# AtomGradient/swift-qwen3-tts

Measured on AMD Instinct MI355X. Metric: codec_tokens_per_s, higher is better.
Workload: dtype bf16

## Files before the change

swift-qwen3-tts_amd/csrc/debug_env.cc:

```cpp
#include <atomic>
#include <cstdlib>
#include <mutex>

#include "kernels.h"

namespace q3 {

namespace {
std::mutex g_mu;
std::atomic<const DebugEnv*> g_env{nullptr};

bool flag(const char* name) { return std::getenv(name) != nullptr; }
int number(const char* name, int dflt) {
    const char* e = std::getenv(name);
    return e && *e ? std::atoi(e) : dflt;
}

const DebugEnv* read_env() {
    DebugEnv* d = new DebugEnv{};
    d->gemm_no_row_split = flag("Q3TTS_GEMM_NO_ROW_SPLIT");
    d->gemm_one_pair = flag("Q3TTS_GEMM_ONE_PAIR");
    d->gemm_parent_forms = number("Q3TTS_GEMM_PARENT_FORMS", 0) != 0;
    d->no_tall_gemm = flag("Q3TTS_NO_TALL_GEMM");
    d->tall_shape = number("Q3TTS_TALL_SHAPE", 0);
    d->chunk_qsplit = number("Q3TTS_CHUNK_QSPLIT", 0);
    d->conv_no_pw = flag("Q3TTS_CONV_NO_PW");
    d->nt_off = std::getenv("Q3TTS_NT") && number("Q3TTS_NT", 1) == 0;
    d->serial_jobs = number("Q3TTS_SERIAL_JOBS", 0) != 0;
    d->fail_back_half = number("Q3TTS_TEST_FAIL_BACK_HALF", 0) != 0;
    d->no_prefix_cache = number("Q3TTS_NO_PREFIX_CACHE", 0) != 0;
    return d;
}
}

const DebugEnv& debug_env() {
    const DebugEnv* e = g_env.load(std::memory_order_acquire);
    if (!e) {
        std::lock_guard<std::mutex> lk(g_mu);
        e = g_env.load(std::memory_order_acquire);
        if (!e) {
            e = read_env();
            g_env.store(e, std::memory_order_release);
        }
    }
    return *e;
}

void debug_env_reload() {
    std::lock_guard<std::mutex> lk(g_mu);
    g_env.store(read_env(), std::memory_order_release);
}

}
```

swift-qwen3-tts_amd/csrc/kernels.h:

```cpp
#pragma once
#include <hip/hip_runtime.h>

#include <cstdint>

namespace q3 {

struct DebugEnv {
    bool gemm_no_row_split;
    bool gemm_one_pair;
    bool gemm_parent_forms;
    bool no_tall_gemm;
    int tall_shape;
    int chunk_qsplit;
    bool conv_no_pw;
    bool nt_off;
    bool serial_jobs;
    bool fail_back_half;
    bool no_prefix_cache;
};
const DebugEnv& debug_env();
void debug_env_reload();

constexpr int kPageTokens = 64;
constexpr int kHeadDim = 128;

struct NormRowsArgs {
    const uint16_t* h;
    int hMB;
    const uint16_t* w;
    float eps;
    uint16_t* out;
    int outMB;
    float* ss_out;
    int M, H;
    const float* ss_in;
    int ss_count, ss_ld;
};
void launch_norm_rows(const NormRowsArgs& a, hipStream_t st);

struct GemmArgs {
    const uint16_t* W;
    const uint32_t* Wsb;
    const uint16_t* x;
    int xMB;
    int M, Mpad, N, K;
    int epi;
    uint16_t* y;
    int ldy;
    int y_tiled, yMB;
    const uint16_t* bias;
    int act_silu;
    const uint16_t* norm_w;
    const float* ss_in;
    int ss_count, ss_ld, norm_dim;
    float norm_eps;
    int nt_weights;
    int resid;
    float* ss_out;
};
void launch_gemm_skinny(const GemmArgs& a, hipStream_t st);
struct SkinnyGeom {
    bool tall;
    int split, mbw;
    int nw, ch, np;
    int gx;
    bool ntw;
    bool tm;
// ... 189 lines not shown
```

swift-qwen3-tts_amd/csrc/kernels/codec_conv.hip:

```cpp
#include <cstdlib>
#include <mutex>

#include "../common.h"
#include "../codec_kernels.h"
#include "../kernels.h"
#include "snake.h"

namespace q3 {
namespace {

constexpr int BM = 128;
constexpr int KC = 32;
constexpr int LDS_LD = 40;
constexpr int MAX_HALO = 56;

__device__ __forceinline__ void st16(float* p, const float4& v) { *reinterpret_cast<float4*>(p) = v; }
__device__ __forceinline__ float4 ld16f(const float* p) { return *reinterpret_cast<const float4*>(p); }

__device__ __forceinline__ float gelu_erf(float v) { return 0.5f * v * (1.0f + erff(v * 0.70710678118654752440f)); }

__device__ __forceinline__ float act_other(float v, int act) {
    switch (act) {
        case 2: return v * 0.5f * (1.0f + tanhf(0.7978845608f * (v + 0.044715f * (v * v * v))));
        case 3: return fmaxf(v, 0.f);
// ... 231 lines not shown
                    for (int c = 0; c < CT; ++c) acc[p][c] = __builtin_amdgcn_mfma_f32_16x16x4f32(wa[g][c].x, xa[g][p].x, acc[p][c], 0, 0, 0);
#pragma unroll
                for (int p = 0; p < 4; ++p)
#pragma unroll
                    for (int c = 0; c < CT; ++c) acc[p][c] = __builtin_amdgcn_mfma_f32_16x16x4f32(wa[g][c].y, xa[g][p].y, acc[p][c], 0, 0, 0);
#pragma unroll
                for (int p = 0; p < 4; ++p)
#pragma unroll
                    for (int c = 0; c < CT; ++c) acc[p][c] = __builtin_amdgcn_mfma_f32_16x16x4f32(wa[g][c].z, xa[g][p].z, acc[p][c], 0, 0, 0);
#pragma unroll
                for (int p = 0; p < 4; ++p)
#pragma unroll
                    for (int c = 0; c < CT; ++c) acc[p][c] = __builtin_amdgcn_mfma_f32_16x16x4f32(wa[g][c].w, xa[g][p].w, acc[p][c], 0, 0, 0);
            }
            buf ^= 1;
        }
    }

    epilogue_tile<CT, true>(a, b, t0 + wm * 64, n0 + wn * (BN / 2), T, lane, acc);
    if (a.out2) snake_pass<CT>(a, smem, b, t0, n0, wn, T, wave, lane, acc, wm);
}

constexpr int ROWH = 40;

typedef _Float16 f16x8 __attribute__((ext_vector_type(8)));
typedef _Float16 f16x4 __attribute__((ext_vector_type(4)));
typedef float f32x4v __attribute__((ext_vector_type(4)));

__device__ __forceinline__ void split_h2(const float4& v, uint2& hi, uint2& lo) {
    const f32x4v x = {v.x, v.y, v.z, v.w};
    const f16x4 h = __builtin_convertvector(x, f16x4);
    const f32x4v r = (x - __builtin_convertvector(h, f32x4v)) * 2048.0f;
    const f16x4 l = __builtin_convertvector(r, f16x4);
    __builtin_memcpy(&hi, &h, 8);
    __builtin_memcpy(&lo, &l, 8);
}

__device__ __forceinline__ f32x4 mfma_f16(const uint4& a, const uint4& b, f32x4 c) {
    f16x8 av, bv;
    __builtin_memcpy(&av, &a, 16);
    __builtin_memcpy(&bv, &b, 16);
    return __builtin_amdgcn_mfma_f32_16x16x32_f16(av, bv, c, 0, 0, 0);
}

__device__ __forceinline__ uint4 f16x8_scale_m11(const uint4& a) {
    f16x8 v;
    __builtin_memcpy(&v, &a, 16);
    v = v * static_cast<_Float16>(0.00048828125f);
    uint4 r;
    __builtin_memcpy(&r, &v, 16);
    return r;
}

template <int CT>
__device__ __forceinline__ void scale_acc(const float* wsc, int N, int n_w, int lane, f32x4 (&acc)[4][CT]) {
    const int nq = n_w + 4 * (lane >> 4);
#pragma unroll
    for (int c = 0; c < CT; ++c) {
        const int n = nq + 16 * c;
        float4 s = make_float4(1.f, 1.f, 1.f, 1.f);
        if (n < N) s = *reinterpret_cast<const float4*>(wsc + n);
#pragma unroll
        for (int p = 0; p < 4; ++p) {
            acc[p][c][0] *= s.x; acc[p][c][1] *= s.y; acc[p][c][2] *= s.z; acc[p][c][3] *= s.w;
        }
    }
}

template <int BN, bool PRO>
__global__ __launch_bounds__(256, 2) void conv_gemm_h2_kernel(ConvGemmArgs a) {
    constexpr int CT = BN / 32;
    extern __shared__ __attribute__((aligned(16))) uint32_t smem3[];
    const int halo = (a.K - 1) * a.dil;
    uint32_t* As = smem3;
    uint32_t* Ws = smem3 + (BM + halo) * ROWH;

    const int tid = threadIdx.x, lane = tid & 63, wave = tid >> 6;
    const int wm = wave >> 1, wn = wave & 1;
    int b, n_tile, m_tile;
    {
        const uint32_t gx = gridDim.x, gy = gridDim.y, nwg = gx * gy * gridDim.z;
        const uint32_t bid = blockIdx.x + gx * (blockIdx.y + gy * blockIdx.z);
        const uint32_t q = nwg >> 3, r = nwg & 7u, xcd = bid & 7u;
        const uint32_t swz = (xcd < r ? xcd * (q + 1) : r * (q + 1) + (xcd - r) * q) + (bid >> 3);
        n_tile = int(swz % gx);
        const uint32_t rest = swz / gx;
        m_tile = int(rest % gy);
        b = int(rest / gy);
    }
    const int n0 = n_tile * BN;
    const int t0 = m_tile * BM;
    const int T = a.frames[b] * a.ppf;
    if (t0 >= T) return;
    const int rows = BM + halo;
    const float* xb = a.x + (size_t)b * a.x_bstride;
    const float* x2b = a.x2;
    const int nchunks = (a.Cin + KC - 1) / KC;
    const int steps = nchunks * a.K;

    f32x4 acc[4][CT];
#pragma unroll
    for (int p = 0; p < 4; ++p)
#pragma unroll
        for (int c = 0; c < CT; ++c) acc[p][c] = f32x4{0.f, 0.f, 0.f, 0.f};

    constexpr int WV = BN * 8 / 256;
    uint4 wreg[WV];
    auto load_w = [&](int step) {
        const int chunk = step / a.K, tap = step % a.K;
        const uint4* src = reinterpret_cast<const uint4*>(a.wh + ((size_t)(tap * nchunks + chunk) * a.N + n0) * 64);
#pragma unroll
        for (int i = 0; i < WV; ++i) {
            const int item = i * 256 + tid;
            uint4 v = make_uint4(0u, 0u, 0u, 0u);
            if (n0 + (item >> 3) < a.N) v = src[item];
            wreg[i] = v;
        }
    };
    auto store_w = [&](int buf) {
#pragma unroll
        for (int i = 0; i < WV; ++i) {
            const int item = i * 256 + tid;
// ... 6 lines not shown
    auto load_a = [&](int chunk) {
        const int c0 = chunk * KC;
#pragma unroll
        for (int i = 0; i < AV; ++i) {
            const int item = i * 256 + tid;
            const int r = item >> 3, c4 = (item & 7) * 4;
            int t = t0 - halo + r;
            if constexpr (PRO) {
                t += a.shift;
                if (a.reflect) t = t < 0 ? -t : (t >= T ? 2 * (T - 1) - t : t);
            }
            float4 v = make_float4(0.f, 0.f, 0.f, 0.f);
            if (r < rows && t >= -a.hist && t < T && c0 + c4 < a.Cin) {
                v = ld16f(xb + (int64_t)t * a.ldx + c0 + c4);
                if constexpr (PRO) {
                    if (x2b) {
                        const float4 u = *reinterpret_cast<const float4*>(x2b + (int64_t)t * a.ldx2 + c0 + c4);
                        v.x += u.x; v.y += u.y; v.z += u.z; v.w += u.w;
                    }
                    if (a.pre_act == 1) {
                        v.x = v.x > 0.f ? v.x : expf(v.x) - 1.0f;
                        v.y = v.y > 0.f ? v.y : expf(v.y) - 1.0f;
                        v.z = v.z > 0.f ? v.z : expf(v.z) - 1.0f;
                        v.w = v.w > 0.f ? v.w : expf(v.w) - 1.0f;
                    }
                    if (a.snake_ea) {
                        const float4 ea = *reinterpret_cast<const float4*>(a.snake_ea + c0 + c4);
                        const float4 ib = *reinterpret_cast<const float4*>(a.snake_ib + c0 + c4);
                        float s;
                        s = sinf(v.x * ea.x); v.x = v.x + ib.x * (s * s);
                        s = sinf(v.y * ea.y); v.y = v.y + ib.y * (s * s);
                        s = sinf(v.z * ea.z); v.z = v.z + ib.z * (s * s);
                        s = sinf(v.w * ea.w); v.w = v.w + ib.w * (s * s);
                    }
                }
            }
            areg[i] = v;
        }
    };
    auto store_a = [&]() {
#pragma unroll
        for (int i = 0; i < AV; ++i) {
            const int item = i * 256 + tid;
            const int r = item >> 3, c4 = (item & 7) * 4;
            if (r >= rows) continue;
            uint2 hi, lo;
            split_h2(areg[i], hi, lo);
            uint32_t* dst = &As[r * ROWH + (c4 >> 1)];
            *reinterpret_cast<uint2*>(dst) = hi;
            *reinterpret_cast<uint2*>(dst + 16) = lo;
        }
    };

    load_w(0);
    load_a(0);
    int buf = 0;
    for (int chunk = 0; chunk < nchunks; ++chunk) {
        __syncthreads();
        store_a();
        if (chunk + 1 < nchunks) load_a(chunk + 1);
        for (int tap = 0; tap < a.K; ++tap) {
            const int step = chunk * a.K + tap;
            store_w(buf);
            __syncthreads();
            if (step + 1 < steps) load_w(step + 1);
            const uint32_t* arow = &As[(wm * 64 + tap * a.dil + (lane & 15)) * ROWH + 4 * (lane >> 4)];
            const uint32_t* wrow = &Ws[(buf * BN + wn * (BN / 2) + (lane & 15)) * ROWH + 4 * (lane >> 4)];
            uint4 xa[2][4], wa[2][CT], wb[CT];
#pragma unroll
            for (int pl = 0; pl < 2; ++pl) {
#pragma unroll
                for (int p = 0; p < 4; ++p) xa[pl][p] = *reinterpret_cast<const uint4*>(arow + p * 16 * ROWH + pl * 16);
#pragma unroll
                for (int c = 0; c < CT; ++c) wa[pl][c] = *reinterpret_cast<const uint4*>(wrow + c * 16 * ROWH + pl * 16);
            }
#pragma unroll
            for (int c = 0; c < CT; ++c) wb[c] = f16x8_scale_m11(wa[0][c]);
#pragma unroll
            for (int p = 0; p < 4; ++p)
#pragma unroll
                for (int c = 0; c < CT; ++c) acc[p][c] = mfma_f16(wb[c], xa[1][p], acc[p][c]);
#pragma unroll
            for (int p = 0; p < 4; ++p)
#pragma unroll
                for (int c = 0; c < CT; ++c) acc[p][c] = mfma_f16(wa[1][c], xa[0][p], acc[p][c]);
#pragma unroll
            for (int p = 0; p < 4; ++p)
#pragma unroll
                for (int c = 0; c < CT; ++c) acc[p][c] = mfma_f16(wa[0][c], xa[0][p], acc[p][c]);
            buf ^= 1;
        }
    }

    scale_acc<CT>(a.wsc, a.N, n0 + wn * (BN / 2), lane, acc);
    if (a.act != 0) epilogue_tile<CT, true>(a, b, t0 + wm * 64, n0 + wn * (BN / 2), T, lane, acc);
    else epilogue_tile<CT, false>(a, b, t0 + wm * 64, n0 + wn * (BN / 2), T, lane, acc);
    if (a.out2) snake_pass<CT>(a, reinterpret_cast<float*>(smem3), b, t0, n0, wn, T, wave, lane, acc, wm);
}

template <int BN, int D>
__global__ __launch_bounds__(256, 2) void conv_pw_h2_kernel(ConvGemmArgs a) {
    constexpr int CT = BN / 32;
    constexpr int WV = BN * 8 / 256, AV = BM * 8 / 256;
    using u32x4 = __attribute__((ext_vector_type(4))) uint32_t;
    using f32x4r = __attribute__((ext_vector_type(4))) float;
    extern __shared__ __attribute__((aligned(16))) uint32_t smem3[];
    uint32_t* As = smem3;
    uint32_t* Ws = smem3 + BM * ROWH;

    const int tid = threadIdx.x, lane = tid & 63, wave = tid >> 6;
    const int wm = wave >> 1, wn = wave & 1;
    int b, n_tile, m_tile;
    {
        const uint32_t gx = gridDim.x, gy = gridDim.y, nwg = gx * gy * gridDim.z;
        const uint32_t bid = blockIdx.x + gx * (blockIdx.y + gy * blockIdx.z);
        const uint32_t q = nwg >> 3, r = nwg & 7u, xcd = bid & 7u;
        const uint32_t swz = (xcd < r ? xcd * (q + 1) : r * (q + 1) + (xcd - r) * q) + (bid >> 3);
        n_tile = int(swz % gx);
        const uint32_t rest = swz / gx;
        m_tile = int(rest % gy);
        b = int(rest / gy);
    }
    const int n0 = n_tile * BN, t0 = m_tile * BM;
    const int T = a.frames[b] * a.ppf;
    if (t0 >= T) return;
    const float* xb = a.x + (size_t)b * a.x_bstride;
    const int steps = (a.Cin + KC - 1) / KC;

    f32x4 acc[4][CT];
#pragma unroll
    for (int p = 0; p < 4; ++p)
#pragma unroll
        for (int c = 0; c < CT; ++c) acc[p][c] = f32x4{0.f, 0.f, 0.f, 0.f};

    const float* asrc[AV];
    bool aok[AV];
#pragma unroll
    for (int i = 0; i < AV; ++i) {
        const int item = i * 256 + tid, r = item >> 3;
        const int t = t0 + r;
        aok[i] = t >= -a.hist && t < T;
        const int tc = t < T ? t : T - 1;
        asrc[i] = xb + (int64_t)tc * a.ldx + (item & 7) * 4;
    }
// ... 35 lines not shown
        _Pragma("unroll") for (int i = 0; i < WV; ++i) {                                          \
            const int item = i * 256 + tid;                                                       \
            *reinterpret_cast<u32x4*>(&Ws[(item >> 3) * ROWH + (item & 7) * 4]) = rw[J][i];       \
        }                                                                                         \
    }
#define Q3_PW_STEP(J, GUARD)                                                                      \
    if (!(GUARD) || s0 + (J) < steps) {                                                           \
        __syncthreads();                     \
        Q3_PW_STORE(J, s0 + (J))                                                                  \
        __builtin_amdgcn_sched_barrier(0);                                                        \
        { const int nx_ = s0 + (J) + D; Q3_PW_LOAD(J, nx_ < steps ? nx_ : steps - 1) }            \
        __builtin_amdgcn_sched_barrier(0);                                                        \
        __syncthreads();                                                                          \
        const uint32_t* arow = &As[(wm * 64 + (lane & 15)) * ROWH + 4 * (lane >> 4)];             \
        const uint32_t* wrow = &Ws[(wn * (BN / 2) + (lane & 15)) * ROWH + 4 * (lane >> 4)];       \
        uint4 xa[2][4], wa[2][CT], wb[CT];                                                        \
        _Pragma("unroll") for (int pl = 0; pl < 2; ++pl) {                                        \
            _Pragma("unroll") for (int p = 0; p < 4; ++p) xa[pl][p] = *reinterpret_cast<const uint4*>(arow + p * 16 * ROWH + pl * 16); \
            _Pragma("unroll") for (int c = 0; c < CT; ++c) wa[pl][c] = *reinterpret_cast<const uint4*>(wrow + c * 16 * ROWH + pl * 16); \
        }                                                                                         \
        _Pragma("unroll") for (int c = 0; c < CT; ++c) wb[c] = f16x8_scale_m11(wa[0][c]);         \
        _Pragma("unroll") for (int p = 0; p < 4; ++p)                                             \
            _Pragma("unroll") for (int c = 0; c < CT; ++c) acc[p][c] = mfma_f16(wb[c], xa[1][p], acc[p][c]);    \
        _Pragma("unroll") for (int p = 0; p < 4; ++p)                                             \
            _Pragma("unroll") for (int c = 0; c < CT; ++c) acc[p][c] = mfma_f16(wa[1][c], xa[0][p], acc[p][c]); \
        _Pragma("unroll") for (int p = 0; p < 4; ++p)                                             \
            _Pragma("unroll") for (int c = 0; c < CT; ++c) acc[p][c] = mfma_f16(wa[0][c], xa[0][p], acc[p][c]); \
    }
#define Q3_PW_GROUP(G)                                       \
    Q3_PW_STEP(0, G) Q3_PW_STEP(1, G)                        \
    if constexpr (D > 2) { Q3_PW_STEP(2, G) }                \
    if constexpr (D > 3) { Q3_PW_STEP(3, G) }

    Q3_PW_LOAD(0, 0)
    __builtin_amdgcn_sched_barrier(0);
    Q3_PW_LOAD(1, 1 < steps ? 1 : steps - 1)
    __builtin_amdgcn_sched_barrier(0);
    if constexpr (D > 2) { Q3_PW_LOAD(2, 2 < steps ? 2 : steps - 1) __builtin_amdgcn_sched_barrier(0); }
    if constexpr (D > 3) { Q3_PW_LOAD(3, 3 < steps ? 3 : steps - 1) __builtin_amdgcn_sched_barrier(0); }
    int s0 = 0;
    for (; s0 + D <= steps; s0 += D) { Q3_PW_GROUP(false) }
    if (s0 < steps) { Q3_PW_GROUP(true) }
#undef Q3_PW_GROUP
#undef Q3_PW_STEP
#undef Q3_PW_STORE
#undef Q3_PW_LOAD

    scale_acc<CT>(a.wsc, a.N, n0 + wn * (BN / 2), lane, acc);
    if (a.act != 0) epilogue_tile<CT, true>(a, b, t0 + wm * 64, n0 + wn * (BN / 2), T, lane, acc);
    else epilogue_tile<CT, false>(a, b, t0 + wm * 64, n0 + wn * (BN / 2), T, lane, acc);
    if (a.out2) snake_pass<CT>(a, reinterpret_cast<float*>(smem3), b, t0, n0, wn, T, wave, lane, acc, wm);
}

template <int CT2, int PT>
__global__ __launch_bounds__(256, 2) void resunit_h2_kernel(ResUnitArgs a) {
    constexpr int C = 16 * CT2, NCH = CT2 / 2, PW = 16 * PT, BMU = 4 * PW;
    constexpr int CG = CT2 >= 12 ? 4 : (CT2 == 6 ? 3 : CT2);
    constexpr int NG = CT2 / CG;
    static_assert(CT2 % CG == 0 && CT2 % 2 == 0, "channel tiles must split into groups and into 32-channel chunks");
    extern __shared__ __attribute__((aligned(16))) uint32_t smem3[];
    const int halo = (a.K - 1) * a.dil;
    uint32_t* As = smem3;
    uint32_t* Ws = smem3 + (BMU + halo) * ROWH;
    const bool wdb = a.wdb != 0;

    const int tid = threadIdx.x, lane = tid & 63, wave = tid >> 6;
    const int b = blockIdx.z;
    const int t0 = blockIdx.y * BMU;
    const int T = a.frames[b] * a.ppf;
    if (t0 >= T) return;
    const int rows = BMU + halo;
    const size_t boff = (size_t)b * a.Tmax * C;
    const float* yb = a.y + boff;
    const int S1 = NCH * a.K;

    f32x4 acc1[PT][CT2];
#pragma unroll
    for (int p = 0; p < PT; ++p)
#pragma unroll
        for (int c = 0; c < CT2; ++c) acc1[p][c] = f32x4{0.f, 0.f, 0.f, 0.f};

    constexpr int WV = (C * 8 + 255) / 256;
    uint4 wreg[WV];
    auto load_w = [&](int step) {
        const uint4* src;
        int items;
        if (step < S1) {
            const int chunk = step / a.K, tap = step % a.K;
            src = reinterpret_cast<const uint4*>(a.w1h + (size_t)(tap * NCH + chunk) * C * 64);
            items = C * 8;
        } else {
            const int j = step - S1, h = j / NCH, m = j % NCH;
            src = reinterpret_cast<const uint4*>(a.w2ph + ((size_t)m * C + h * CG * 16) * 64);
            items = CG * 16 * 8;
        }
#pragma unroll
        for (int i = 0; i < WV; ++i) {
            const int item = i * 256 + tid;
            wreg[i] = item < items ? src[item] : make_uint4(0u, 0u, 0u, 0u);
        }
    };
    auto store_w = [&](int buf, int items) {
#pragma unroll
        for (int i = 0; i < WV; ++i) {
            const int item = i * 256 + tid;
            if (item < items) *reinterpret_cast<uint4*>(&Ws[(buf * C + (item >> 3)) * ROWH + (item & 7) * 4]) = wreg[i];
        }
    };

    constexpr int AV = ((BMU + MAX_HALO) * 8 + 255) / 256;
    float4 areg[AV];
    auto load_a = [&](int chunk) {
        const int c0 = chunk * KC;
#pragma unroll
        for (int i = 0; i < AV; ++i) {
            const int item = i * 256 + tid;
            const int r = item >> 3, c4 = (item & 7) * 4;
            const int t = t0 - halo + r;
            float4 v = make_float4(0.f, 0.f, 0.f, 0.f);
            if (r < rows && t >= -a.hist && t < T) v = ld16f(yb + (int64_t)t * C + c0 + c4);
            areg[i] = v;
        }
    };
    auto store_a = [&](int chunk) {
        const int c0 = chunk * KC, c4 = (tid & 7) * 4;
        const float4 ea = *reinterpret_cast<const float4*>(a.ea1 + c0 + c4);
        const float4 ib = *reinterpret_cast<const float4*>(a.ib1 + c0 + c4);
#pragma unroll
        for (int i = 0; i < AV; ++i) {
            const int item = i * 256 + tid;
            const int r = item >> 3;
            if (r >= rows) continue;
            const int t = t0 - halo + r;
            float4 v = areg[i];
            if (t >= -a.hist && t < T) {
                v.x = v.x + ib.x * snake_sin2(v.x * ea.x);
                v.y = v.y + ib.y * snake_sin2(v.y * ea.y);
                v.z = v.z + ib.z * snake_sin2(v.z * ea.z);
                v.w = v.w + ib.w * snake_sin2(v.w * ea.w);
            }
            uint2 hi, lo;
            split_h2(v, hi, lo);
            uint32_t* dst = &As[r * ROWH + (c4 >> 1)];
            *reinterpret_cast<uint2*>(dst) = hi;
            *reinterpret_cast<uint2*>(dst + 16) = lo;
        }
    };

    load_w(0);
    load_a(0);
    int buf = 0;
    for (int chunk = 0; chunk < NCH; ++chunk) {
        __syncthreads();
        store_a(chunk);
        if (chunk + 1 < NCH) load_a(chunk + 1);
        for (int tap = 0; tap < a.K; ++tap) {
            const int step = chunk * a.K + tap;
            if (!wdb && tap > 0) __syncthreads();
            store_w(buf, C * 8);
            __syncthreads();
            load_w(step + 1);
            const uint32_t* arow = &As[(PW * wave + tap * a.dil + (lane & 15)) * ROWH + 4 * (lane >> 4)];
            const uint32_t* wrow = &Ws[(buf * C + (lane & 15)) * ROWH + 4 * (lane >> 4)];
            uint4 xa[2][PT];
#pragma unroll
            for (int pl = 0; pl < 2; ++pl)
#pragma unroll
                for (int p = 0; p < PT; ++p) xa[pl][p] = *reinterpret_cast<const uint4*>(arow + p * 16 * ROWH + pl * 16);
#pragma unroll
            for (int g = 0; g < NG; ++g) {
                uint4 wa[2][CG], wb[CG];
#pragma unroll
                for (int pl = 0; pl < 2; ++pl)
#pragma unroll
                    for (int c = 0; c < CG; ++c) wa[pl][c] = *reinterpret_cast<const uint4*>(wrow + (g * CG + c) * 16 * ROWH + pl * 16);
#pragma unroll
                for (int c = 0; c < CG; ++c) wb[c] = f16x8_scale_m11(wa[0][c]);
#pragma unroll
                for (int p = 0; p < PT; ++p)
#pragma unroll
                    for (int c = 0; c < CG; ++c) acc1[p][g * CG + c] = mfma_f16(wb[c], xa[1][p], acc1[p][g * CG + c]);
#pragma unroll
                for (int p = 0; p < PT; ++p)
#pragma unroll
                    for (int c = 0; c < CG; ++c) acc1[p][g * CG + c] = mfma_f16(wa[1][c], xa[0][p], acc1[p][g * CG + c]);
#pragma unroll
                for (int p = 0; p < PT; ++p)
#pragma unroll
                    for (int c = 0; c < CG; ++c) acc1[p][g * CG + c] = mfma_f16(wa[0][c], xa[0][p], acc1[p][g * CG + c]);
            }
            if (wdb) buf ^= 1;
        }
    }

    const int q4 = 4 * (lane >> 4);
    int big = 0;
#pragma unroll
    for (int c = 0; c < CT2; ++c) {
        const float4 sv = *reinterpret_cast<const float4*>(a.wsc1 + 16 * c + q4);
        const float4 bv = a.b1 ? *reinterpret_cast<const float4*>(a.b1 + 16 * c + q4) : make_float4(0.f, 0.f, 0.f, 0.f);
        const float4 ea = *reinterpret_cast<const float4*>(a.ea2 + 16 * c + q4);
        const float e[4] = {ea.x, ea.y, ea.z, ea.w}, bb[4] = {bv.x, bv.y, bv.z, bv.w}, ss[4] = {sv.x, sv.y, sv.z, sv.w};
#pragma unroll
        for (int p = 0; p < PT; ++p)
#pragma unroll
            for (int j = 0; j < 4; ++j) {
                acc1[p][c][j] = acc1[p][c][j] * ss[j] + bb[j];
                big |= !(fabsf(acc1[p][c][j] * e[j]) < 1.0e6f);
            }
    }
    if (__syncthreads_or(big)) {
        float4* stash = reinterpret_cast<float4*>(As) + wave * (CT2 * 64);
#pragma unroll
        for (int p = 0; p < PT; ++p) {
#pragma unroll
            for (int c = 0; c < CT2; ++c) stash[c * 64 + lane] = make_float4(acc1[p][c][0], acc1[p][c][1], acc1[p][c][2], acc1[p][c][3]);
#pragma unroll 1
            for (int c = 0; c < CT2; ++c) {
                float4 v = stash[c * 64 + lane];
                const float4 ea = *reinterpret_cast<const float4*>(a.ea2 + 16 * c + q4);
                const float4 ib = *reinterpret_cast<const float4*>(a.ib2 + 16 * c + q4);
                v.x = v.x + ib.x * snake_sin2(v.x * ea.x);
                v.y = v.y + ib.y * snake_sin2(v.y * ea.y);
                v.z = v.z + ib.z * snake_sin2(v.z * ea.z);
                v.w = v.w + ib.w * snake_sin2(v.w * ea.w);
                stash[c * 64 + lane] = v;
            }
#pragma unroll
            for (int c = 0; c < CT2; ++c) {
                const float4 v = stash[c * 64 + lane];
                acc1[p][c] = f32x4{v.x, v.y, v.z, v.w};
            }
        }
        __syncthreads();
    } else {
#pragma unroll
        for (int c = 0; c < CT2; ++c) {
            const float4 ea = *reinterpret_cast<const float4*>(a.ea2 + 16 * c + q4);
            const float4 ib = *reinterpret_cast<const float4*>(a.ib2 + 16 * c + q4);
            const float e[4] = {ea.x, ea.y, ea.z, ea.w}, ii[4] = {ib.x, ib.y, ib.z, ib.w};
#pragma unroll
            for (int p = 0; p < PT; ++p)
#pragma unroll
                for (int j = 0; j < 4; ++j) acc1[p][c][j] = acc1[p][c][j] + ii[j] * snake_sin2_poly(acc1[p][c][j] * e[j]);
        }
    }

    const uint32_t* wrow2 = &Ws[(lane & 15) * ROWH + 4 * (lane >> 4)];
    float4* stash = reinterpret_cast<float4*>(As) + wave * (CG * 64);
#pragma unroll
    for (int h = 0; h < NG; ++h) {
        f32x4 acc2[PT][CG];
#pragma unroll
        for (int p = 0; p < PT; ++p)
#pragma unroll
            for (int c = 0; c < CG; ++c) acc2[p][c] = f32x4{0.f, 0.f, 0.f, 0.f};
#pragma unroll
        for (int m = 0; m < NCH; ++m) {
            const int j = h * NCH + m;
            if (j > 0) __syncthreads();
            store_w(0, CG * 16 * 8);
            __syncthreads();
            if (j + 1 < NG * NCH) load_w(S1 + j + 1);
            uint4 xb[2][PT], wa[2][CG], wb[CG];
#pragma unroll
            for (int p = 0; p < PT; ++p) {
                const float4 v0 = make_float4(acc1[p][2 * m][0], acc1[p][2 * m][1], acc1[p][2 * m][2], acc1[p][2 * m][3]);
                const float4 v1 = make_float4(acc1[p][2 * m + 1][0], acc1[p][2 * m + 1][1], acc1[p][2 * m + 1][2], acc1[p][2 * m + 1][3]);
                uint2 h0, l0, h1, l1;
                split_h2(v0, h0, l0);
                split_h2(v1, h1, l1);
                xb[0][p] = make_uint4(h0.x, h0.y, h1.x, h1.y);
                xb[1][p] = make_uint4(l0.x, l0.y, l1.x, l1.y);
            }
#pragma unroll
            for (int pl = 0; pl < 2; ++pl)
#pragma unroll
                for (int c = 0; c < CG; ++c) wa[pl][c] = *reinterpret_cast<const uint4*>(wrow2 + c * 16 * ROWH + pl * 16);
#pragma unroll
            for (int c = 0; c < CG; ++c) wb[c] = f16x8_scale_m11(wa[0][c]);
#pragma unroll
            for (int p = 0; p < PT; ++p)
#pragma unroll
                for (int c = 0; c < CG; ++c) acc2[p][c] = mfma_f16(wb[c], xb[1][p], acc2[p][c]);
#pragma unroll
            for (int p = 0; p < PT; ++p)
#pragma unroll
                for (int c = 0; c < CG; ++c) acc2[p][c] = mfma_f16(wa[1][c], xb[0][p], acc2[p][c]);
#pragma unroll
            for (int p = 0; p < PT; ++p)
#pragma unroll
                for (int c = 0; c < CG; ++c) acc2[p][c] = mfma_f16(wa[0][c], xb[0][p], acc2[p][c]);
        }
        float4 rvs[PT][CG], bv2[CG], sv2[CG];
#pragma unroll
        for (int c = 0; c < CG; ++c) {
            const int n = 16 * (h * CG + c) + q4;
            bv2[c] = a.b2 ? *reinterpret_cast<const float4*>(a.b2 + n) : make_float4(0.f, 0.f, 0.f, 0.f);
            sv2[c] = *reinterpret_cast<const float4*>(a.wsc2 + n);
        }
#pragma unroll
        for (int p = 0; p < PT; ++p) {
            const int t = t0 + PW * wave + 16 * p + (lane & 15);
#pragma unroll
            for (int c = 0; c < CG; ++c) {
                rvs[p][c] = make_float4(0.f, 0.f, 0.f, 0.f);
                if (t < T) rvs[p][c] = *reinterpret_cast<const float4*>(yb + (size_t)t * C + 16 * (h * CG + c) + q4);
            }
        }
#pragma unroll
        for (int p = 0; p < PT; ++p) {
            const int t = t0 + PW * wave + 16 * p + (lane & 15);
#pragma unroll
            for (int c = 0; c < CG; ++c) {
                const int n = 16 * (h * CG + c) + q4;
                const float4 rv = rvs[p][c], bv = bv2[c], sv = sv2[c];
                float4 v = make_float4(acc2[p][c][0] * sv.x + rv.x, acc2[p][c][1] * sv.y + rv.y, acc2[p][c][2] * sv.z + rv.z,
                                       acc2[p][c][3] * sv.w + rv.w);
                if (a.b2)
                    v = make_float4((acc2[p][c][0] * sv.x + bv.x) + rv.x, (acc2[p][c][1] * sv.y + bv.y) + rv.y,
                                    (acc2[p][c][2] * sv.z + bv.z) + rv.z, (acc2[p][c][3] * sv.w + bv.w) + rv.w);
                if (t < T) st16(a.out + boff + (size_t)t * C + n, v);
                acc2[p][c] = f32x4{v.x, v.y, v.z, v.w};
            }
        }
        if (a.out2) {
#pragma unroll
            for (int p = 0; p < PT; ++p) {
#pragma unroll
                for (int c = 0; c < CG; ++c) stash[c * 64 + lane] = make_float4(acc2[p][c][0], acc2[p][c][1], acc2[p][c][2], acc2[p][c][3]);
                const int t = t0 + PW * wave + 16 * p + (lane & 15);
// ... 29 lines not shown
    const int bmu = a.C == 96 ? 256 : 128;
    const int rows = bmu + (a.K - 1) * a.dil;
    d.family = ConvDispatch::RESUNIT_H2;
    d.BN = a.C;
    d.CT2 = a.C / 16;
    d.PT = bmu / 64;
    d.wdb = size_t(rows + 2 * a.C) * ROWH * sizeof(uint32_t) <= 80 * 1024 ? 1 : 0;
    d.lds = size_t(rows + (d.wdb ? 2 : 1) * a.C) * ROWH * sizeof(uint32_t);
    d.gx = 1; d.gy = unsigned((a.Tmax + bmu - 1) / bmu); d.gz = unsigned(a.B);
    return d;
}

constexpr int PWD = 2;

ConvDispatch conv_gemm_dispatch(const ConvGemmArgs& a) {
    Q3_CHECK((a.K - 1) * a.dil <= MAX_HALO, 3, "conv_gemm: receptive field too large");
    Q3_CHECK(!a.x2 || (a.B == 1 && a.ldx2 % 4 == 0), 3, "conv_gemm: the pre-add input is single-row only");
    Q3_CHECK(a.Cin % 4 == 0 && a.N % 4 == 0 && a.ldx % 4 == 0 && a.ldo % 4 == 0, 3, "conv_gemm: channels must be multiples of 4");
    Q3_CHECK(!a.out2 || (a.post_ea && a.post_ib && a.post_C > 0 && a.post_C % 4 == 0), 3, "conv_gemm: activated output without its parameters");
    ConvDispatch d;
    const int mt = (a.Tmax + BM - 1) / BM;
    if (mt <= 0 || a.B <= 0) return d;
    int BN = 64;
    if (a.N % 128 == 0) BN = 128;
    else if (a.N % 96 == 0) BN = 96;
    else if (a.N > 128 && (a.N % 64) != 0) BN = 128;
    d.BN = BN;
    d.gx = unsigned((a.N + BN - 1) / BN); d.gy = unsigned(mt); d.gz = unsigned(a.B);
    if (a.wh) {
        Q3_CHECK(a.wsc != nullptr, 3, "conv_gemm: fp16x2 weights without their row scales");
        const bool pro = a.x2 || a.pre_act || a.snake_ea || a.shift || a.reflect;
        if (!pro && a.K == 1 && !debug_env().conv_no_pw) {
            d.family = ConvDispatch::PW_H2;
            d.pw_depth = PWD;
            d.lds = size_t(BM + BN) * ROWH * sizeof(uint32_t);
        } else {
            d.family = ConvDispatch::H2;
            d.pro = pro ? 1 : 0;
            d.lds = size_t(BM + (a.K - 1) * a.dil + 2 * BN) * ROWH * sizeof(uint32_t);
        }
    } else {
        d.family = ConvDispatch::F32;
        d.lds = size_t(BM + (a.K - 1) * a.dil + 2 * BN) * LDS_LD * sizeof(float);
    }
    return d;
}

void launch_resunit(const ResUnitArgs& a0, hipStream_t st) {
    static std::once_flag attr_once[kMaxDevices];
    ResUnitArgs a = a0;
    const ConvDispatch d = resunit_dispatch(a);
    if (!d.gx) return;
    std::call_once(device_once(attr_once), [] {
        void (*ks[4])(ResUnitArgs) = {&resunit_h2_kernel<2, 2>, &resunit_h2_kernel<4, 2>, &resunit_h2_kernel<6, 4>, &resunit_h2_kernel<12, 2>};
        for (auto k : ks)
            Q3_HIP(hipFuncSetAttribute(reinterpret_cast<const void*>(k), hipFuncAttributeMaxDynamicSharedMemorySize, 80 * 1024));
    });
    a.wdb = d.wdb;
    const dim3 grid(d.gx, d.gy, d.gz), block(256);
    switch (d.CT2) {
        case 2: hipLaunchKernelGGL((resunit_h2_kernel<2, 2>), grid, block, d.lds, st, a); break;
        case 4: hipLaunchKernelGGL((resunit_h2_kernel<4, 2>), grid, block, d.lds, st, a); break;
        case 6: hipLaunchKernelGGL((resunit_h2_kernel<6, 4>), grid, block, d.lds, st, a); break;
        default: hipLaunchKernelGGL((resunit_h2_kernel<12, 2>), grid, block, d.lds, st, a); break;
    }
}

void launch_conv_gemm(const ConvGemmArgs& a, hipStream_t st) {
    static std::once_flag attr_once[kMaxDevices];
    const ConvDispatch d = conv_gemm_dispatch(a);
    if (!d.gx) return;
    const dim3 grid(d.gx, d.gy, d.gz), block(256);
    std::call_once(device_once(attr_once), [] {
        Q3_HIP(hipFuncSetAttribute(reinterpret_cast<const void*>(&conv_gemm_kernel<128>), hipFuncAttributeMaxDynamicSharedMemorySize, 80 * 1024));
        Q3_HIP(hipFuncSetAttribute(reinterpret_cast<const void*>(&conv_gemm_kernel<96>), hipFuncAttributeMaxDynamicSharedMemorySize, 80 * 1024));
        Q3_HIP(hipFuncSetAttribute(reinterpret_cast<const void*>(&conv_gemm_kernel<64>), hipFuncAttributeMaxDynamicSharedMemorySize, 80 * 1024));
        void (*h2_kernels[6])(ConvGemmArgs) = {&conv_gemm_h2_kernel<128, true>, &conv_gemm_h2_kernel<128, false>,
                                                &conv_gemm_h2_kernel<96, true>,  &conv_gemm_h2_kernel<96, false>,
                                                &conv_gemm_h2_kernel<64, true>,  &conv_gemm_h2_kernel<64, false>};
        for (auto k : h2_kernels)
            Q3_HIP(hipFuncSetAttribute(reinterpret_cast<const void*>(k), hipFuncAttributeMaxDynamicSharedMemorySize, 80 * 1024));
    });
    auto go = [&](void (*kern)(ConvGemmArgs)) { hipLaunchKernelGGL(kern, grid, block, d.lds, st, a); };
    switch (d.family) {
        case ConvDispatch::PW_H2:
            switch (d.BN) {
                case 128: go(&conv_pw_h2_kernel<128, PWD>); break;
                case 96: go(&conv_pw_h2_kernel<96, PWD>); break;
                default: go(&conv_pw_h2_kernel<64, PWD>); break;
            }
            break;
        case ConvDispatch::H2:
            switch (d.BN) {
                case 128: d.pro ? go(&conv_gemm_h2_kernel<128, true>) : go(&conv_gemm_h2_kernel<128, false>); break;
                case 96: d.pro ? go(&conv_gemm_h2_kernel<96, true>) : go(&conv_gemm_h2_kernel<96, false>); break;
                default: d.pro ? go(&conv_gemm_h2_kernel<64, true>) : go(&conv_gemm_h2_kernel<64, false>); break;
            }
            break;
        default:
            switch (d.BN) {
                case 128: go(&conv_gemm_kernel<128>); break;
                case 96: go(&conv_gemm_kernel<96>); break;
                default: go(&conv_gemm_kernel<64>); break;
            }
    }
}

}
```

Baseline: 10650.

## Restructure codec conv kernels' weight/activation pipelining with precomputed offsets and W2 double-buffering

Adds a new default path (PF=false) to the half-precision conv GEMM and resunit kernels. Weight loads use precomputed per-thread byte offsets, the per-tap weight tile is double-buffered in LDS with a flipping offset, and activation fragments are reloaded across taps, which removes some barriers and address math. In the resunit second conv, W2 tiles alternate between two LDS regions to drop a barrier, and split activations are cached in registers across groups instead of being recomputed. The old path stays reachable through Q3TTS_CONV_PARENT_FORMS; the exchange is higher register pressure and larger code.

```diff
diff --git a/swift-qwen3-tts_amd/csrc/debug_env.cc b/swift-qwen3-tts_amd/csrc/debug_env.cc
--- a/swift-qwen3-tts_amd/csrc/debug_env.cc
+++ b/swift-qwen3-tts_amd/csrc/debug_env.cc
@@ -25,6 +25,7 @@
     d->tall_shape = number("Q3TTS_TALL_SHAPE", 0);
     d->chunk_qsplit = number("Q3TTS_CHUNK_QSPLIT", 0);
     d->conv_no_pw = flag("Q3TTS_CONV_NO_PW");
+    d->conv_parent_forms = number("Q3TTS_CONV_PARENT_FORMS", 0) != 0;
     d->nt_off = std::getenv("Q3TTS_NT") && number("Q3TTS_NT", 1) == 0;
     d->serial_jobs = number("Q3TTS_SERIAL_JOBS", 0) != 0;
     d->fail_back_half = number("Q3TTS_TEST_FAIL_BACK_HALF", 0) != 0;
diff --git a/swift-qwen3-tts_amd/csrc/kernels.h b/swift-qwen3-tts_amd/csrc/kernels.h
--- a/swift-qwen3-tts_amd/csrc/kernels.h
+++ b/swift-qwen3-tts_amd/csrc/kernels.h
@@ -13,6 +13,7 @@
     int tall_shape;
     int chunk_qsplit;
     bool conv_no_pw;
+    bool conv_parent_forms;
     bool nt_off;
     bool serial_jobs;
     bool fail_back_half;
diff --git a/swift-qwen3-tts_amd/csrc/kernels/codec_conv.hip b/swift-qwen3-tts_amd/csrc/kernels/codec_conv.hip
--- a/swift-qwen3-tts_amd/csrc/kernels/codec_conv.hip
+++ b/swift-qwen3-tts_amd/csrc/kernels/codec_conv.hip
@@ -307,6 +307,12 @@
     return r;
 }
 
+__device__ __forceinline__ uint4 ld16u_at(const uint4* base, uint32_t byte_off) {
+    typedef uint32_t u32x4 __attribute__((ext_vector_type(4)));
+    const u32x4 v = *reinterpret_cast<const u32x4*>(reinterpret_cast<const char*>(base) + byte_off);
+    return make_uint4(v.x, v.y, v.z, v.w);
+}
+
 template <int CT>
 __device__ __forceinline__ void scale_acc(const float* wsc, int N, int n_w, int lane, f32x4 (&acc)[4][CT]) {
     const int nq = n_w + 4 * (lane >> 4);
@@ -322,7 +328,7 @@
     }
 }
 
-template <int BN, bool PRO>
+template <int BN, bool PRO, bool PF>
 __global__ __launch_bounds__(256, 2) void conv_gemm_h2_kernel(ConvGemmArgs a) {
     constexpr int CT = BN / 32;
     extern __shared__ __attribute__((aligned(16))) uint32_t smem3[];
@@ -435,6 +441,7 @@
         }
     };
 
+    if constexpr (PF) {
     load_w(0);
     load_a(0);
     int buf = 0;
@@ -473,6 +480,146 @@
                 for (int c = 0; c < CT; ++c) acc[p][c] = mfma_f16(wa[0][c], xa[0][p], acc[p][c]);
             buf ^= 1;
         }
+    }
+    } else {
+    const uint32_t wtile = uint32_t(a.N) * 8u;
+    const size_t wtap = size_t(nchunks) * wtile;
+    const uint4* wchunk = reinterpret_cast<const uint4*>(a.wh) + size_t(n0) * 8;
+    uint32_t woff[WV];
+#pragma unroll
+    for (int i = 0; i < WV; ++i) {
+        const int item = i * 256 + tid, n = n0 + (item >> 3);
+        woff[i] = uint32_t((n < a.N ? item : (a.N - 1 - n0) * 8 + (item & 7)) * 16);
+    }
+    auto load_wp = [&](const uint4* src) {
+#pragma unroll
+        for (int i = 0; i < WV; ++i) wreg[i] = ld16u_at(src, woff[i]);
+    };
+    const int r0 = tid >> 3, c4 = (tid & 7) * 4;
+    uint32_t amask = 0, smask = 0;
+    int trow[PRO ? AV : 1];
+#pragma unroll
+    for (int i = 0; i < AV; ++i) {
+        const int r = r0 + 32 * i;
+        int t = t0 - halo + r;
+        if constexpr (PRO) {
+            t += a.shift;
+            if (a.reflect) t = t < 0 ? -t : (t >= T ? 2 * (T - 1) - t : t);
+            trow[i] = t;
+        }
+        smask |= uint32_t(r < rows) << i;
+        amask |= uint32_t(r < rows && t >= -a.hist && t < T) << i;
+    }
+    const float* ap0 = xb + (int64_t)(t0 - halo + r0) * a.ldx + c4;
+    const int64_t astride = 32 * (int64_t)a.ldx;
+    auto load_ap = [&](int c0) {
+        const bool cok = c0 + c4 < a.Cin;
+#pragma unroll
+        for (int i = 0; i < AV; ++i) {
+            float4 v = make_float4(0.f, 0.f, 0.f, 0.f);
+            if (((amask >> i) & 1u) && cok) {
+                if constexpr (!PRO) {
+                    v = ld16f(ap0 + i * astride + c0);
+                } else {
+                    v = ld16f(xb + (int64_t)trow[i] * a.ldx + c0 + c4);
+                    if (x2b) {
+                        const float4 u = *reinterpret_cast<const float4*>(x2b + (int64_t)trow[i] * a.ldx2 + c0 + c4);
+                        v.x += u.x; v.y += u.y; v.z += u.z; v.w += u.w;
+                    }
+                    if (a.pre_act == 1) {
+                        v.x = v.x > 0.f ? v.x : expf(v.x) - 1.0f;
+                        v.y = v.y > 0.f ? v.y : expf(v.y) - 1.0f;
+                        v.z = v.z > 0.f ? v.z : expf(v.z) - 1.0f;
+                        v.w = v.w > 0.f ? v.w : expf(v.w) - 1.0f;
+                    }
+                    if (a.snake_ea) {
+                        const float4 ea = *reinterpret_cast<const float4*>(a.snake_ea + c0 + c4);
+                        const float4 ib = *reinterpret_cast<const float4*>(a.snake_ib + c0 + c4);
+                        float s;
+                        s = sinf(v.x * ea.x); v.x = v.x + ib.x * (s * s);
+                        s = sinf(v.y * ea.y); v.y = v.y + ib.y * (s * s);
+                        s = sinf(v.z * ea.z); v.z = v.z + ib.z * (s * s);
+                        s = sinf(v.w * ea.w); v.w = v.w + ib.w * (s * s);
+                    }
+                }
+            }
+            areg[i] = v;
+        }
+    };
+    uint32_t* adst = &As[r0 * ROWH + (c4 >> 1)];
+    auto store_ap = [&]() {
+#pragma unroll
+        for (int i = 0; i < AV; ++i) {
+            if (!((smask >> i) & 1u)) continue;
+            uint2 hi, lo;
+            split_h2(areg[i], hi, lo);
+            *reinterpret_cast<uint2*>(adst + i * 32 * ROWH) = hi;
+            *reinterpret_cast<uint2*>(adst + i * 32 * ROWH + 16) = lo;
+        }
+    };
+    const uint32_t* arow0 = &As[(wm * 64 + (lane & 15)) * ROWH + 4 * (lane >> 4)];
+    const uint32_t* wrow0 = &Ws[(wn * (BN / 2) + (lane & 15)) * ROWH + 4 * (lane >> 4)];
+    uint32_t* wdst = &Ws[(tid >> 3) * ROWH + (tid & 7) * 4];
+    const int dstep = a.dil * ROWH;
+    const int K = a.K;
+
+    load_wp(wchunk);
+    load_ap(0);
+    int bofs = 0;
+    uint4 xa[2][4];
+    for (int chunk = 0; chunk < nchunks; ++chunk) {
+        __syncthreads();
+        store_ap();
+        if (chunk + 1 < nchunks) load_ap((chunk + 1) * KC);
+        const uint32_t* arow = arow0;
+        const uint4* wcur = wchunk;
+        for (int tap = 0; tap < K; ++tap) {
+#pragma unroll
+            for (int i = 0; i < WV; ++i) *reinterpret_cast<uint4*>(wdst + bofs + i * 32 * ROWH) = wreg[i];
+            if (tap > 0) {
+#pragma unroll
+                for (int p = 0; p < 4; ++p) xa[0][p] = *reinterpret_cast<const uint4*>(arow + p * 16 * ROWH);
+            }
+            __syncthreads();
+            const bool last_tap = tap + 1 == K;
+            const uint4* wnext = last_tap ? wchunk + wtile : wcur + wtap;
+            if (!last_tap || chunk + 1 < nchunks) load_wp(wnext);
+            wcur = wnext;
+            if (tap == 0) {
+#pragma unroll
+                for (int pl = 0; pl < 2; ++pl)
+#pragma unroll
+                    for (int p = 0; p < 4; ++p) xa[pl][p] = *reinterpret_cast<const uint4*>(arow + p * 16 * ROWH + pl * 16);
+            }
+            const uint32_t* wrow = wrow0 + bofs;
+            uint4 wa[2][CT], wb[CT];
+#pragma unroll
+            for (int pl = 0; pl < 2; ++pl)
+#pragma unroll
+                for (int c = 0; c < CT; ++c) wa[pl][c] = *reinterpret_cast<const uint4*>(wrow + c * 16 * ROWH + pl * 16);
+#pragma unroll
+            for (int c = 0; c < CT; ++c) {
+                wb[c] = f16x8_scale_m11(wa[0][c]);
+#pragma unroll
+                for (int p = 0; p < 4; ++p) acc[p][c] = mfma_f16(wb[c], xa[1][p], acc[p][c]);
+            }
+            arow += dstep;
+            if (!last_tap) {
+#pragma unroll
+                for (int p = 0; p < 4; ++p) xa[1][p] = *reinterpret_cast<const uint4*>(arow + p * 16 * ROWH + 16);
+            }
+#pragma unroll
+            for (int p = 0; p < 4; ++p)
+#pragma unroll
+                for (int c = 0; c < CT; ++c) acc[p][c] = mfma_f16(wa[1][c], xa[0][p], acc[p][c]);
+#pragma unroll
+            for (int p = 0; p < 4; ++p)
+#pragma unroll
+                for (int c = 0; c < CT; ++c) acc[p][c] = mfma_f16(wa[0][c], xa[0][p], acc[p][c]);
+            bofs = BN * ROWH - bofs;
+        }
+        wchunk += wtile;
+    }
     }
 
     scale_acc<CT>(a.wsc, a.N, n0 + wn * (BN / 2), lane, acc);
@@ -614,7 +761,7 @@
     if (a.out2) snake_pass<CT>(a, reinterpret_cast<float*>(smem3), b, t0, n0, wn, T, wave, lane, acc, wm);
 }
 
-template <int CT2, int PT>
+template <int CT2, int PT, bool PF>
 __global__ __launch_bounds__(256, 2) void resunit_h2_kernel(ResUnitArgs a) {
     constexpr int C = 16 * CT2, NCH = CT2 / 2, PW = 16 * PT, BMU = 4 * PW;
     constexpr int CG = CT2 >= 12 ? 4 : (CT2 == 6 ? 3 : CT2);
@@ -709,6 +856,141 @@
         }
     };
 
+    constexpr int W2ROWS = CG * 16, W2ITEMS = W2ROWS * 8;
+    constexpr int W2SECOND = 2 * W2ROWS <= C ? W2ROWS : C;
+    const bool two = 2 * W2ROWS <= C || wdb;
+    auto load_w2 = [&](int j) {
+        const uint4* src = reinterpret_cast<const uint4*>(a.w2ph + ((size_t)(j % NCH) * C + (j / NCH) * CG * 16) * 64);
+#pragma unroll
+        for (int i = 0; i < WV; ++i)
+            if (i * 256 < W2ITEMS) wreg[i] = (i + 1) * 256 <= W2ITEMS || i * 256 + tid < W2ITEMS ? src[i * 256 + tid] : make_uint4(0u, 0u, 0u, 0u);
+    };
+    auto store_w2 = [&](int row0) {
+#pragma unroll
+        for (int i = 0; i < WV; ++i)
+            if (i * 256 < W2ITEMS && ((i + 1) * 256 <= W2ITEMS || i * 256 + tid < W2ITEMS))
+                *reinterpret_cast<uint4*>(&Ws[(row0 + (tid >> 3) + 32 * i) * ROWH + (tid & 7) * 4]) = wreg[i];
+    };
+    if constexpr (!PF) {
+    static_assert((C * 8) % 256 == 0, "conv1's weight tile is a whole number of pieces per thread");
+    const int K = a.K;
+    const uint4* wchunk = reinterpret_cast<const uint4*>(a.w1h);
+    uint32_t woff[WV];
+#pragma unroll
+    for (int i = 0; i < WV; ++i) woff[i] = uint32_t(i * 256 + tid) * 16u;
+    auto load_w1 = [&](const uint4* src) {
+#pragma unroll
+        for (int i = 0; i < WV; ++i) wreg[i] = ld16u_at(src, woff[i]);
+    };
+    const int r0 = tid >> 3, c4 = (tid & 7) * 4;
+    uint32_t amask = 0, smask = 0;
+#pragma unroll
+    for (int i = 0; i < AV; ++i) {
+        const int r = r0 + 32 * i, t = t0 - halo + r;
+        smask |= uint32_t(r < rows) << i;
+        amask |= uint32_t(r < rows && t >= -a.hist && t < T) << i;
+    }
+    const float* ap0 = yb + (int64_t)(t0 - halo + r0) * C + c4;
+    auto load_ap = [&](int c0) {
+#pragma unroll
+        for (int i = 0; i < AV; ++i) {
+            float4 v = make_float4(0.f, 0.f, 0.f, 0.f);
+            if ((amask >> i) & 1u) v = ld16f(ap0 + i * 32 * C + c0);
+            areg[i] = v;
+        }
+    };
+    uint32_t* adst = &As[r0 * ROWH + (c4 >> 1)];
+    auto store_ap = [&](int c0) {
+        const float4 ea = *reinterpret_cast<const float4*>(a.ea1 + c0 + c4);
+        const float4 ib = *reinterpret_cast<const float4*>(a.ib1 + c0 + c4);
+#pragma unroll
+        for (int i = 0; i < AV; ++i) {
+            if (!((smask >> i) & 1u)) continue;
+            float4 v = areg[i];
+            if ((amask >> i) & 1u) {
+                v.x = v.x + ib.x * snake_sin2(v.x * ea.x);
+                v.y = v.y + ib.y * snake_sin2(v.y * ea.y);
+                v.z = v.z + ib.z * snake_sin2(v.z * ea.z);
+                v.w = v.w + ib.w * snake_sin2(v.w * ea.w);
+            }
+            uint2 hi, lo;
+            split_h2(v, hi, lo);
+            *reinterpret_cast<uint2*>(adst + i * 32 * ROWH) = hi;
+            *reinterpret_cast<uint2*>(adst + i * 32 * ROWH + 16) = lo;
+        }
+    };
+    const uint32_t* arow0 = &As[(PW * wave + (lane & 15)) * ROWH + 4 * (lane >> 4)];
+    const uint32_t* wrow0 = &Ws[(lane & 15) * ROWH + 4 * (lane >> 4)];
+    uint32_t* wdst = &Ws[(tid >> 3) * ROWH + (tid & 7) * 4];
+    const int dstep = a.dil * ROWH;
+    const int bflip = wdb ? C * ROWH : 0;
+
+    load_w1(wchunk);
+    load_ap(0);
+    int bofs = 0;
+    uint4 xa[2][PT];
+    for (int chunk = 0; chunk < NCH; ++chunk) {
+        __syncthreads();
+        store_ap(chunk * KC);
+        if (chunk + 1 < NCH) load_ap((chunk + 1) * KC);
+        const uint32_t* arow = arow0;
+        const uint4* wcur = wchunk;
+        for (int tap = 0; tap < K; ++tap) {
+            if (tap > 0) {
+#pragma unroll
+                for (int p = 0; p < PT; ++p) xa[0][p] = *reinterpret_cast<const uint4*>(arow + p * 16 * ROWH);
+                if (!wdb) __syncthreads();
+            }
+#pragma unroll
+            for (int i = 0; i < WV; ++i) *reinterpret_cast<uint4*>(wdst + bofs + i * 32 * ROWH) = wreg[i];
+            __syncthreads();
+            const bool last_tap = tap + 1 == K;
+            if (last_tap && chunk + 1 == NCH) {
+                load_w2(0);
+            } else {
+                const uint4* wnext = last_tap ? wchunk + C * 8 : wcur + NCH * C * 8;
+                load_w1(wnext);
+                wcur = wnext;
+            }
+            if (tap == 0) {
+#pragma unroll
+                for (int pl = 0; pl < 2; ++pl)
+#pragma unroll
+                    for (int p = 0; p < PT; ++p) xa[pl][p] = *reinterpret_cast<const uint4*>(arow + p * 16 * ROWH + pl * 16);
+            }
+            const uint32_t* wrow = wrow0 + bofs;
+            arow += dstep;
+#pragma unroll
+            for (int g = 0; g < NG; ++g) {
+                uint4 wa[2][CG], wb[CG];
+#pragma unroll
+                for (int pl = 0; pl < 2; ++pl)
+#pragma unroll
+                    for (int c = 0; c < CG; ++c) wa[pl][c] = *reinterpret_cast<const uint4*>(wrow + (g * CG + c) * 16 * ROWH + pl * 16);
+#pragma unroll
+                for (int c = 0; c < CG; ++c) {
+                    wb[c] = f16x8_scale_m11(wa[0][c]);
+#pragma unroll
+                    for (int p = 0; p < PT; ++p) acc1[p][g * CG + c] = mfma_f16(wb[c], xa[1][p], acc1[p][g * CG + c]);
+                }
+                if (g == NG - 1 && !last_tap) {
+#pragma unroll
+                    for (int p = 0; p < PT; ++p) xa[1][p] = *reinterpret_cast<const uint4*>(arow + p * 16 * ROWH + 16);
+                }
+#pragma unroll
+                for (int p = 0; p < PT; ++p)
+#pragma unroll
+                    for (int c = 0; c < CG; ++c) acc1[p][g * CG + c] = mfma_f16(wa[1][c], xa[0][p], acc1[p][g * CG + c]);
+#pragma unroll
+                for (int p = 0; p < PT; ++p)
+#pragma unroll
+                    for (int c = 0; c < CG; ++c) acc1[p][g * CG + c] = mfma_f16(wa[0][c], xa[0][p], acc1[p][g * CG + c]);
+            }
+            bofs = bflip - bofs;
+        }
+        wchunk += C * 8;
+    }
+    } else {
     load_w(0);
     load_a(0);
     int buf = 0;
@@ -754,6 +1036,7 @@
             if (wdb) buf ^= 1;
         }
     }
+    }
 
     const int q4 = 4 * (lane >> 4);
     int big = 0;
@@ -810,6 +1093,7 @@
 
     const uint32_t* wrow2 = &Ws[(lane & 15) * ROWH + 4 * (lane >> 4)];
     float4* stash = reinterpret_cast<float4*>(As) + wave * (CG * 64);
+    uint4 xh2[PT][NCH], xl2[PT][NCH];
 #pragma unroll
     for (int h = 0; h < NG; ++h) {
         f32x4 acc2[PT][CG];
@@ -820,25 +1104,44 @@
 #pragma unroll
         for (int m = 0; m < NCH; ++m) {
             const int j = h * NCH + m;
-            if (j > 0) __syncthreads();
-            store_w(0, CG * 16 * 8);
-            __syncthreads();
-            if (j + 1 < NG * NCH) load_w(S1 + j + 1);
+            int wofs2 = 0;
+            if constexpr (PF) {
+                if (j > 0) __syncthreads();
+                store_w(0, CG * 16 * 8);
+                __syncthreads();
+                if (j + 1 < NG * NCH) load_w(S1 + j + 1);
+            } else {
+                if (j > 0 && !two) __syncthreads();
+                const int row0 = (two && (j & 1)) ? W2SECOND : 0;
+                store_w2(row0);
+                __syncthreads();
+                if (j + 1 < NG * NCH) load_w2(j + 1);
+                wofs2 = row0 * ROWH;
+            }
             uint4 xb[2][PT], wa[2][CG], wb[CG];
 #pragma unroll
             for (int p = 0; p < PT; ++p) {
-                const float4 v0 = make_float4(acc1[p][2 * m][0], acc1[p][2 * m][1], acc1[p][2 * m][2], acc1[p][2 * m][3]);
-                const float4 v1 = make_float4(acc1[p][2 * m + 1][0], acc1[p][2 * m + 1][1], acc1[p][2 * m + 1][2], acc1[p][2 * m + 1][3]);
-                uint2 h0, l0, h1, l1;
-                split_h2(v0, h0, l0);
-                split_h2(v1, h1, l1);
-                xb[0][p] = make_uint4(h0.x, h0.y, h1.x, h1.y);
-                xb[1][p] = make_uint4(l0.x, l0.y, l1.x, l1.y);
+                if (PF || h == 0) {
+                    const float4 v0 = make_float4(acc1[p][2 * m][0], acc1[p][2 * m][1], acc1[p][2 * m][2], acc1[p][2 * m][3]);
+                    const float4 v1 = make_float4(acc1[p][2 * m + 1][0], acc1[p][2 * m + 1][1], acc1[p][2 * m + 1][2], acc1[p][2 * m + 1][3]);
+                    uint2 h0, l0, h1, l1;
+                    split_h2(v0, h0, l0);
+                    split_h2(v1, h1, l1);
+                    xb[0][p] = make_uint4(h0.x, h0.y, h1.x, h1.y);
+                    xb[1][p] = make_uint4(l0.x, l0.y, l1.x, l1.y);
+                    if constexpr (!PF) {
+                        xh2[p][m] = xb[0][p];
+                        xl2[p][m] = xb[1][p];
+                    }
+                } else {
+                    xb[0][p] = xh2[p][m];
+                    xb[1][p] = xl2[p][m];
+                }
             }
 #pragma unroll
             for (int pl = 0; pl < 2; ++pl)
 #pragma unroll
-                for (int c = 0; c < CG; ++c) wa[pl][c] = *reinterpret_cast<const uint4*>(wrow2 + c * 16 * ROWH + pl * 16);
+                for (int c = 0; c < CG; ++c) wa[pl][c] = *reinterpret_cast<const uint4*>(wrow2 + wofs2 + c * 16 * ROWH + pl * 16);
 #pragma unroll
             for (int c = 0; c < CG; ++c) wb[c] = f16x8_scale_m11(wa[0][c]);
 #pragma unroll
@@ -974,17 +1277,21 @@
     const ConvDispatch d = resunit_dispatch(a);
     if (!d.gx) return;
     std::call_once(device_once(attr_once), [] {
-        void (*ks[4])(ResUnitArgs) = {&resunit_h2_kernel<2, 2>, &resunit_h2_kernel<4, 2>, &resunit_h2_kernel<6, 4>, &resunit_h2_kernel<12, 2>};
+        void (*ks[8])(ResUnitArgs) = {&resunit_h2_kernel<2, 2, false>, &resunit_h2_kernel<4, 2, false>, &resunit_h2_kernel<6, 4, false>,
+                                      &resunit_h2_kernel<12, 2, false>, &resunit_h2_kernel<2, 2, true>, &resunit_h2_kernel<4, 2, true>,
+                                      &resunit_h2_kernel<6, 4, true>, &resunit_h2_kernel<12, 2, true>};
         for (auto k : ks)
             Q3_HIP(hipFuncSetAttribute(reinterpret_cast<const void*>(k), hipFuncAttributeMaxDynamicSharedMemorySize, 80 * 1024));
     });
     a.wdb = d.wdb;
     const dim3 grid(d.gx, d.gy, d.gz), block(256);
+    auto go = [&](void (*kern)(ResUnitArgs)) { hipLaunchKernelGGL(kern, grid, block, d.lds, st, a); };
+    const bool pf = debug_env().conv_parent_forms;
     switch (d.CT2) {
-        case 2: hipLaunchKernelGGL((resunit_h2_kernel<2, 2>), grid, block, d.lds, st, a); break;
-        case 4: hipLaunchKernelGGL((resunit_h2_kernel<4, 2>), grid, block, d.lds, st, a); break;
-        case 6: hipLaunchKernelGGL((resunit_h2_kernel<6, 4>), grid, block, d.lds, st, a); break;
-        default: hipLaunchKernelGGL((resunit_h2_kernel<12, 2>), grid, block, d.lds, st, a); break;
+        case 2: pf ? go(&resunit_h2_kernel<2, 2, true>) : go(&resunit_h2_kernel<2, 2, false>); break;
+        case 4: pf ? go(&resunit_h2_kernel<4, 2, true>) : go(&resunit_h2_kernel<4, 2, false>); break;
+        case 6: pf ? go(&resunit_h2_kernel<6, 4, true>) : go(&resunit_h2_kernel<6, 4, false>); break;
+        default: pf ? go(&resunit_h2_kernel<12, 2, true>) : go(&resunit_h2_kernel<12, 2, false>); break;
     }
 }
 
@@ -997,9 +1304,11 @@
         Q3_HIP(hipFuncSetAttribute(reinterpret_cast<const void*>(&conv_gemm_kernel<128>), hipFuncAttributeMaxDynamicSharedMemorySize, 80 * 1024));
         Q3_HIP(hipFuncSetAttribute(reinterpret_cast<const void*>(&conv_gemm_kernel<96>), hipFuncAttributeMaxDynamicSharedMemorySize, 80 * 1024));
         Q3_HIP(hipFuncSetAttribute(reinterpret_cast<const void*>(&conv_gemm_kernel<64>), hipFuncAttributeMaxDynamicSharedMemorySize, 80 * 1024));
-        void (*h2_kernels[6])(ConvGemmArgs) = {&conv_gemm_h2_kernel<128, true>, &conv_gemm_h2_kernel<128, false>,
-                                                &conv_gemm_h2_kernel<96, true>,  &conv_gemm_h2_kernel<96, false>,
-                                                &conv_gemm_h2_kernel<64, true>,  &conv_gemm_h2_kernel<64, false>};
+        void (*h2_kernels[11])(ConvGemmArgs) = {
+            &conv_gemm_h2_kernel<128, true, false>, &conv_gemm_h2_kernel<128, false, false>, &conv_gemm_h2_kernel<96, true, false>,
+            &conv_gemm_h2_kernel<64, true, false>,  &conv_gemm_h2_kernel<64, false, false>,
+            &conv_gemm_h2_kernel<128, true, true>,  &conv_gemm_h2_kernel<128, false, true>,  &conv_gemm_h2_kernel<96, true, true>,
+            &conv_gemm_h2_kernel<96, false, true>,  &conv_gemm_h2_kernel<64, true, true>,    &conv_gemm_h2_kernel<64, false, true>};
         for (auto k : h2_kernels)
             Q3_HIP(hipFuncSetAttribute(reinterpret_cast<const void*>(k), hipFuncAttributeMaxDynamicSharedMemorySize, 80 * 1024));
     });
@@ -1012,13 +1321,21 @@
                 default: go(&conv_pw_h2_kernel<64, PWD>); break;
             }
             break;
-        case ConvDispatch::H2:
+        case ConvDispatch::H2: {
+            const bool pf = debug_env().conv_parent_forms;
+#define Q3_H2(BN_) (d.pro ? (pf ? go(&conv_gemm_h2_kernel<BN_, true, true>) : go(&conv_gemm_h2_kernel<BN_, true, false>)) \
+                          : (pf ? go(&conv_gemm_h2_kernel<BN_, false, true>) : go(&conv_gemm_h2_kernel<BN_, false, false>)))
             switch (d.BN) {
-                case 128: d.pro ? go(&conv_gemm_h2_kernel<128, true>) : go(&conv_gemm_h2_kernel<128, false>); break;
-                case 96: d.pro ? go(&conv_gemm_h2_kernel<96, true>) : go(&conv_gemm_h2_kernel<96, false>); break;
-                default: d.pro ? go(&conv_gemm_h2_kernel<64, true>) : go(&conv_gemm_h2_kernel<64, false>); break;
-            }
+                case 128: Q3_H2(128); break;
+                case 96:
+                    if (!d.pro) go(&conv_gemm_h2_kernel<96, false, true>);
+                    else pf ? go(&conv_gemm_h2_kernel<96, true, true>) : go(&conv_gemm_h2_kernel<96, true, false>);
+                    break;
+                default: Q3_H2(64); break;
+            }
+#undef Q3_H2
             break;
+        }
         default:
             switch (d.BN) {
                 case 128: go(&conv_gemm_kernel<128>); break;
```

Result: slower. 10330 (-2.9%).
